# ay-lab/fithic

Measured on AMD Instinct MI355X. Metric: contact-pairs/sec through spline+p-value+BH pass (5 kb cis, whole node), higher is better.
Workload: dtype f64

## Files before the change

### fithic_amd/csrc/fhx_ctx.hpp

```cpp
#pragma once
#include <hip/hip_runtime.h>

#include <atomic>
#include <functional>
#include <chrono>
#include <thread>
#include <memory>
#include <sys/stat.h>
#include <unistd.h>
#include <deque>
#include <mutex>
#include <map>
#include <condition_variable>
#include <algorithm>
#include <climits>
#include <cstddef>
#include <cmath>
#include <cstdio>
#include <cstdlib>
#include <cstring>
#include <string>
#include <vector>

#include "../../include/fithic_mi355x.h"
// ... 42 lines not shown
    const int32_t* loc2;
    const int32_t* count;
    const double* slot_bias;
    bool no_bias;
    const double* prior_lut;
    int lut_len;
    dev::BinomTables intra, inter;
    double inter_chr_prob;
    double outlier_thres;
    int lo_idx, hi_idx;
    int mode;
    int64_t n;
    double* p;
    unsigned long long* top_hist;
    uint8_t* outlier;
    int nonfixed;
    const int32_t* slot_mid;
    const double* table_x;
    const double* table_y;
    int n_table;
    double min_x, max_x;
    long long dist_low, dist_up;
    double total_intra, total_inter;
};

constexpr int K2_THREADS = 256;

constexpr int K2_QUEUES = dev::BC_COUNT - 1;

struct QEntry {
    unsigned int row;
    int count;
    double prior;
};

constexpr int K2_MAX_SHARDS = 2048;

struct QSpan {
    QEntry* base;
    long long cap_s;
    int dir;
    int n_shards;
    const unsigned long long* count;
};
__device__ __forceinline__ QEntry* qentry(const QSpan& q, int shard, long long j) {
    return q.base + (long long)shard * q.cap_s + (long long)q.dir * j;
}

struct K2Queues {
    QSpan q[K2_QUEUES + 1];
    unsigned long long* count;
    unsigned int* heavy_hist;
};

constexpr int K2H_BUCKETS = 2048;
constexpr int K2H_BLOCKS = 1024;
__device__ __forceinline__ int k2h_bucket(int signed_count);

struct CutoffToHost {
    volatile unsigned long long* words = nullptr;
    unsigned long long ticket = 0;
    unsigned int* done = nullptr;
    unsigned long long* zero_me = nullptr;
};

constexpr int K3_DENSE_PERCENT = 35;
constexpr int K2_COUNTER_WORDS = 8;
constexpr int FDR_BUCKETS = 51;

struct DeviceWords {
    unsigned long long bh_kept;
    unsigned long long bh_cutoff;
    unsigned long long bh_below;
    unsigned long long array_kept;
    unsigned long long array_cutoff;
    unsigned long long sort_n;
    unsigned long long run_total;
    unsigned long long nf_keys;
    unsigned long long outliers_added;
    unsigned long long first_dup;
    unsigned long long memo_overflow;
    alignas(128) unsigned long long k2_redo;
    unsigned long long k2_next[K2_COUNTER_WORDS - 1];
    alignas(128) unsigned long long k3_dense;
    alignas(128) unsigned long long fdr_buckets[FDR_BUCKETS];
};
static_assert(offsetof(DeviceWords, k2_next) == offsetof(DeviceWords, k2_redo) + sizeof(unsigned long long) &&
                  sizeof(DeviceWords::k2_next) == (K2_COUNTER_WORDS - 1) * sizeof(unsigned long long),
              "k2_closed zeroes K2_COUNTER_WORDS words starting at k2_redo");
static_assert(K2_COUNTER_WORDS >= 2 + K2_QUEUES, "k2_next holds k2h_heavy's word and one per class queue");
static_assert(sizeof(DeviceWords::fdr_buckets) == FDR_BUCKETS * sizeof(unsigned long long), "one word per FDR bucket");

constexpr int K2_CL_ITEMS = 4;
constexpr int K2_CL_TILE = K2_THREADS * K2_CL_ITEMS;

constexpr int K2_CLOSED = K2_QUEUES + 1;
constexpr int K2_CLOSED_LOCAL = K2_QUEUES + 2;
constexpr int K2_CLASSES = K2_QUEUES + 2;

constexpr int K2H_KCAP = 1023;
constexpr int K2H_GENERIC = 2 * K2H_KCAP;
constexpr int K2H_THREADS = 256;
constexpr int K2H_MAX_ROWS = 4;

constexpr int SORT_THREADS = 256;
constexpr int SORT_WAVES = SORT_THREADS / 64;
constexpr int SORT_ITEMS = 16;
constexpr int SORT_TILE = SORT_THREADS * SORT_ITEMS;
constexpr int CP_THREADS = 1024;
constexpr int CP_WAVES = CP_THREADS / 64;
constexpr int CP_ITEMS = 16;
constexpr int CP_TILE = CP_THREADS * CP_ITEMS;
constexpr int CP_STRIP = 2048;
constexpr int SORT_BLOCKS = 1024;
constexpr int RADIX_BITS = 11;
constexpr int RADIX = 1 << RADIX_BITS;
constexpr int SORT_PASSES = 6;
constexpr int SORT_BITS_LARGE = 8;

constexpr int TOP_SHIFT = 50;
constexpr int TOP_BINS = 8192;

__device__ __forceinline__ unsigned long long pvalue_key(double v) {
    unsigned long long bits = (unsigned long long)__double_as_longlong(v);
    if (bits == 0x8000000000000000ull) bits = 0ull;
    return bits;
}

constexpr unsigned long long KEY_ONE = 0x3FF0000000000000ull;
constexpr unsigned long long KEY_KEEP_ALL = 0x7FF0000000000001ull;

constexpr int SCAT_ITEMS = 8;
constexpr int BH_THREADS = 256;
constexpr int BH_ITEMS = 8;
constexpr int BH_TILE = BH_THREADS * BH_ITEMS;
constexpr int SEG_THREADS = 256;
constexpr int SEG_ITEMS = 16;
constexpr int SEG_TILE = SEG_THREADS * SEG_ITEMS;

}

using namespace fhx;

namespace fhx {
struct DistState;
struct K3Host;
}

struct FhxPinnedPair;
void fhx_pinned_pair_free(FhxPinnedPair* p);

struct SideWorkers {
    std::thread th[2];
    std::mutex mu;
    std::condition_variable cv;
    std::function<void()> job[2];
    bool busy[2] = {false, false}, quit = false, started = false;
    void start() {
        if (started) return;
        started = true;
        for (int k = 0; k < 2; ++k)
            th[k] = std::thread([this, k] {
                std::unique_lock<std::mutex> g(mu);
                for (;;) {
                    cv.wait(g, [&] { return quit || busy[k]; });
                    if (quit) return;
                    std::function<void()> f = std::move(job[k]);
                    g.unlock();
                    f();
                    g.lock();
                    busy[k] = false;
                    cv.notify_all();
                }
// ... 310 lines not shown
```

### fithic_amd/csrc/fhx_k2.hip

```cpp
#include "fhx_ctx.hpp"

namespace fhx {

__device__ __forceinline__ double prior_by_search(const K2Params& P, long long dist) {
    double look = (double)dist;
    if (look < P.min_x) look = P.min_x;
    if (look > P.max_x) look = P.max_x;
    int lo = 0, hi = P.n_table;
    while (lo < hi) {
        const int mid = (lo + hi) >> 1;
        if (P.table_x[mid] < look)
            lo = mid + 1;
        else
            hi = mid;
    }
    return P.table_y[min(lo, P.n_table - 1)];
}

template <int NF = -1>
__device__ __forceinline__ bool row_prior(const K2Params& P, int l1, int l2, double& prior, bool& is_inter) {
    const bool inter = l2 < 0;
    const int s2 = inter ? ~l2 : l2;
    const double b1 = P.no_bias ? 1.0 : P.slot_bias[l1], b2 = P.no_bias ? 1.0 : P.slot_bias[s2];
    if ((b1 < 0 || b2 < 0) && !inter) return false;
// ... 212 lines not shown
            unsigned int mine[2] = {0u, 0u};
            unsigned int shift_of[ITEMS];
#pragma unroll
            for (int r = 0; r < ITEMS; ++r) {
                const int k = cls_of[r] - 1;
                const int f = k >= 3 ? k - 3 : k;
                shift_of[r] = 10u * (unsigned int)(f < 0 ? 0 : f);
                const unsigned int one = k >= 0 ? (1u << shift_of[r]) : 0u;
                mine[0] += k < 3 ? one : 0u;
                mine[1] += k >= 3 ? one : 0u;
            }
            const unsigned int incl0 = wave_incl_sum_u32(mine[0]), incl1 = wave_incl_sum_u32(mine[1]);
            const unsigned int all0 = (unsigned int)__builtin_amdgcn_readlane((int)incl0, 63), all1 = (unsigned int)__builtin_amdgcn_readlane((int)incl1, 63);
            tot[0] = all0 & 1023u; tot[1] = (all0 >> 10) & 1023u; tot[2] = (all0 >> 20) & 1023u;
            tot[3] = all1 & 1023u; tot[4] = (all1 >> 10) & 1023u; tot[5] = (all1 >> 20) & 1023u;
            unsigned int run[2] = {incl0 - mine[0], incl1 - mine[1]};
#pragma unroll
            for (int r = 0; r < ITEMS; ++r) {
                const int k = cls_of[r] - 1;
                const unsigned int word = k >= 3 ? run[1] : run[0];
                before_cls[r] = (word >> shift_of[r]) & 1023u;
                const unsigned int one = k >= 0 ? (1u << shift_of[r]) : 0u;
                run[0] += k < 3 ? one : 0u;
                run[1] += k >= 3 ? one : 0u;
            }
        } else {
#pragma unroll
            for (int r = 0; r < ITEMS; ++r) {
                before_cls[r] = 0;
#pragma unroll
                for (int k = 1; k <= K2_CLASSES; ++k) {
                    const unsigned long long m = __ballot(cls_of[r] == k);
                    if (cls_of[r] == k) before_cls[r] = tot[k - 1] + (unsigned int)__popcll(m & lane_lt);
                    tot[k - 1] += (unsigned int)__popcll(m);
                }
            }
        }
        const unsigned int my_tot = lane == 0 ? tot[0] : (lane == 1 ? tot[1] : (lane == 2 ? tot[2] : (lane == 3 ? tot[3] : tot[4])));
        unsigned int my_base = 0;
        if (lane <= K2_QUEUES && my_tot) my_base = atomicAdd(&cnt[lane], my_tot);
        unsigned int wave_base[K2_QUEUES + 1];
#pragma unroll
        for (int k = 0; k <= K2_QUEUES; ++k) wave_base[k] = __shfl(my_base, k, 64);
#pragma unroll
        for (int r = 0; r < ITEMS; ++r) {
            const int k = cls_of[r] - 1;
            if (k >= 0 && k <= K2_QUEUES) {
                const unsigned int wb = k == 0 ? wave_base[0] : (k == 1 ? wave_base[1] : (k == 2 ? wave_base[2] : (k == 3 ? wave_base[3] : wave_base[4])));
                QEntry e;
                e.row = (unsigned int)(row0 + r);
                e.count = count_of[r];
                e.prior = prior_of[r];
                *qentry(Q.q[k], shard, (long long)(wb + before_cls[r])) = e;
                if (k == dev::BC_CF_SWAPPED - 1 && count_heavy) atomicAdd(&heavy_lds[k2h_bucket(e.count)], 1u);
            } else if (cls_of[r] == K2_CLOSED_LOCAL) {
                cf_prior[wave][before_cls[r]] = prior_of[r];
                cf_idx[wave][before_cls[r]] = (unsigned short)((lane * ITEMS + r) | (count_of[r] < 0 ? 0x8000 : 0));
            }
        }
        __builtin_amdgcn_fence(__ATOMIC_RELEASE, "wavefront");
        __builtin_amdgcn_wave_barrier();
        __builtin_amdgcn_fence(__ATOMIC_ACQUIRE, "wavefront");
        const unsigned int n_local = tot[K2_CLASSES - 1];
        for (unsigned int j = lane; j < n_local; j += 64) {
            const unsigned int ix = cf_idx[wave][j];
            const double n_total = (ix & 0x8000u) ? P.inter.n : P.intra.n;
            const double pr = cf_prior[wave][j];
            const double pv = -dev::cephes_expm1(n_total * dev::cephes_log1p(-pr));
            P.p[wave_row0 + (ix & 0x7FFFu)] = pv;
            H.add(pv);
        }
        __builtin_amdgcn_fence(__ATOMIC_RELEASE, "wavefront");
        __builtin_amdgcn_wave_barrier();
    }
    __syncthreads();
    if (threadIdx.x <= K2_QUEUES) Q.count[(size_t)threadIdx.x * K2_MAX_SHARDS + shard] = cnt[threadIdx.x];
    if (count_heavy)
        for (int d = threadIdx.x; d < K2H_BUCKETS; d += K2_THREADS)
            if (heavy_lds[d]) atomicAdd(&Q.heavy_hist[(size_t)d * K2H_BLOCKS + (shard & (K2H_BLOCKS - 1))], heavy_lds[d]);
    H.flush(P.top_hist);
}

__global__ __launch_bounds__(K2_THREADS) void k2_closed(K2Params P, QSpan q, unsigned long long* __restrict__ zero_words,
                                                        unsigned long long* __restrict__ cutoff_word) {
    __shared__ unsigned int hist_lds[K2_HIST_BINS];
    if (blockIdx.x == 0 && threadIdx.x < K2_COUNTER_WORDS) zero_words[threadIdx.x] = 0ull;
    if (blockIdx.x == 0 && threadIdx.x == K2_COUNTER_WORDS) *cutoff_word = KEY_KEEP_ALL;
    FusedHist H;
    H.init(hist_lds, P.top_hist);
    for (int sh = blockIdx.x; sh < q.n_shards; sh += gridDim.x) {
        const long long n = (long long)q.count[sh];
        for (long long j = threadIdx.x; j < n; j += blockDim.x) {
            const QEntry e = *qentry(q, sh, j);
            const double pv = dev::bdtrc_closed_form(e.count < 0 ? P.inter.n : P.intra.n, e.prior);
            store_p<false>(P.p + e.row, pv);
            H.add(pv);
        }
    }
    H.flush(P.top_hist);
}

struct QDense {
    static constexpr int PAIRS = K2_MAX_SHARDS / 2;
    unsigned int* prefix;
    const unsigned long long* count;
    __device__ __forceinline__ void build(const QSpan& q, unsigned int* prefix_lds, unsigned int* wave_tot) {
        static_assert(PAIRS % K2_THREADS == 0, "whole pairs per thread");
        constexpr int PER = PAIRS / K2_THREADS;
        prefix = prefix_lds;
        count = q.count;
        unsigned int c[PER], s = 0;
#pragma unroll
        for (int k = 0; k < PER; ++k) {
            const int sh = 2 * ((int)threadIdx.x * PER + k);
            c[k] = (sh < q.n_shards ? (unsigned int)q.count[sh] : 0u) + (sh + 1 < q.n_shards ? (unsigned int)q.count[sh + 1] : 0u);
            s += c[k];
        }
        const unsigned int incl = wave_incl_sum_u32(s);
        if ((threadIdx.x & 63) == 63) wave_tot[threadIdx.x >> 6] = incl;
        __syncthreads();
        unsigned int run = incl - s;
        for (int w = 0; w < (int)(threadIdx.x >> 6); ++w) run += wave_tot[w];
#pragma unroll
        for (int k = 0; k < PER; ++k) {
            prefix_lds[threadIdx.x * PER + k] = run;
            run += c[k];
        }
        if (threadIdx.x == K2_THREADS - 1) prefix_lds[PAIRS] = run;
        __syncthreads();
    }
    __device__ __forceinline__ unsigned int total() const { return prefix[PAIRS]; }
    __device__ __forceinline__ int pair_of(unsigned int v) const {
        int lo = 0, hi = PAIRS;
#pragma unroll 1
        while (hi - lo > 1) {
            const int mid = (lo + hi) >> 1;
            if (prefix[mid] <= v)
                lo = mid;
            else
                hi = mid;
        }
        return lo;
    }
    struct Cursor {
        int pr;
        unsigned int base, end, c0;
    };
    __device__ __forceinline__ void load(Cursor& c) const {
        c.base = prefix[c.pr];
        c.end = prefix[c.pr + 1];
        c.c0 = (unsigned int)count[2 * c.pr];
    }
    __device__ __forceinline__ Cursor open(unsigned int v) const {
        Cursor c;
        c.pr = pair_of(v);
        load(c);
        return c;
    }
    __device__ __forceinline__ const QEntry* at(const QSpan& q, Cursor& c, unsigned int v) const {
        if (v >= c.end) {
            do ++c.pr;
            while (v >= prefix[c.pr + 1]);
            load(c);
        }
        const unsigned int u = v - c.base;
        return u < c.c0 ? qentry(q, 2 * c.pr, (long long)u) : qentry(q, 2 * c.pr + 1, (long long)(u - c.c0));
    }
};
constexpr int K2_WAVES = K2_THREADS / 64;

// ... 19 lines not shown
        const bool is_inter = e.count < 0;
        const int c = is_inter ? -e.count : e.count;
        const double pv = dev::bdtrc_count_class<CLS, SMALL_N>(c, is_inter ? P.inter : P.intra, e.prior);
        store_p<false>(P.p + e.row, pv);
        H.add(pv);
    }
    H.flush(P.top_hist);
}

constexpr int K2_SORT_TILE = 1024;
constexpr int K2_SORT_BUCKETS = 32;
template <int CLS, bool SMALL_N, int WPE>
__global__ __launch_bounds__(K2_THREADS) __attribute__((amdgpu_waves_per_eu(WPE))) void k2_queue_by_count(K2Params P, QSpan q,
                                                                                                         unsigned int* next_tile) {
    static_assert(K2_SORT_TILE == 4 * K2_THREADS, "four entries per thread");
    __shared__ QEntry tile[K2_SORT_TILE];
    __shared__ unsigned int bucket_cnt[K2_SORT_BUCKETS], bucket_off[K2_SORT_BUCKETS];
    __shared__ unsigned int hist_lds[K2_HIST_BINS];
    __shared__ unsigned int prefix_lds[QDense::PAIRS + 1], wave_tot[K2_WAVES], tile_lds;
    FusedHist H;
    H.init(hist_lds, P.top_hist);
    QDense D;
    D.build(q, prefix_lds, wave_tot);
    const unsigned int total = D.total();
    const unsigned int share = (total + gridDim.x - 1) / gridDim.x;
    const unsigned int rounds = max(1u, (share + K2_SORT_TILE - 1) / K2_SORT_TILE);
    const unsigned int tile_n = max(min((unsigned int)K2_SORT_TILE, ((share + rounds - 1) / rounds + 63u) & ~63u), 64u);
    const unsigned int tiles = (total + tile_n - 1) / tile_n;
    unsigned int mine = blockIdx.x;
    for (;;) {
        if (threadIdx.x < K2_SORT_BUCKETS) bucket_cnt[threadIdx.x] = 0;
        if (threadIdx.x == 0) tile_lds = mine;
        __syncthreads();
        const unsigned int t = tile_lds;
        if (t >= tiles) break;
        if (threadIdx.x == 0) mine = gridDim.x + atomicAdd(next_tile, 1u);
        const unsigned int v0 = t * tile_n;
        const int m = (int)min(tile_n, total - v0);
        QEntry e[4];
        int bucket[4];
        unsigned int slot[4];
        QDense::Cursor cur{0, 0u, 0u, 0u};
        if ((int)threadIdx.x < m) cur = D.open(v0 + threadIdx.x);
#pragma unroll
        for (int r = 0; r < 4; ++r) {
            const int idx = r * K2_THREADS + (int)threadIdx.x;
            bucket[r] = -1;
            if (idx < m) {
                e[r] = *D.at(q, cur, v0 + idx);
                const int c = e[r].count < 0 ? -e[r].count : e[r].count;
                bucket[r] = c < K2_SORT_BUCKETS - 1 ? c : K2_SORT_BUCKETS - 1;
                slot[r] = atomicAdd(&bucket_cnt[bucket[r]], 1u);
            }
        }
        __syncthreads();
        if (threadIdx.x < K2_SORT_BUCKETS) {
            unsigned int off = 0;
            for (int b = 0; b < (int)threadIdx.x; ++b) off += bucket_cnt[b];
            bucket_off[threadIdx.x] = off;
        }
        __syncthreads();
#pragma unroll
        for (int r = 0; r < 4; ++r)
            if (bucket[r] >= 0) tile[bucket_off[bucket[r]] + slot[r]] = e[r];
        __syncthreads();
#pragma unroll 1
        for (int r = 0; r < 4; ++r) {
            const int idx = r * K2_THREADS + threadIdx.x;
            if (idx < m) {
                const QEntry x = tile[idx];
                const bool is_inter = x.count < 0;
                const int c = is_inter ? -x.count : x.count;
                const double pv = dev::bdtrc_count_class<CLS, SMALL_N>(c, is_inter ? P.inter : P.intra, x.prior);
                store_p<false>(P.p + x.row, pv);
                H.add(pv);
            }
        }
        __syncthreads();
    }
    H.flush(P.top_hist);
}



__device__ __forceinline__ int k2h_bucket(int signed_count) {
    const bool inter = signed_count < 0;
    const int c = inter ? -signed_count : signed_count;
    return c < K2H_KCAP ? (inter ? K2H_KCAP + c : c) : K2H_GENERIC;
}

__global__ __launch_bounds__(K2H_THREADS) void k2h_scatter(QSpan q, const unsigned int* __restrict__ block_hist,
                                                           const unsigned int* __restrict__ off, QEntry* __restrict__ out) {
    __shared__ unsigned int cursor[K2H_BUCKETS];
    for (int d = threadIdx.x; d < K2H_BUCKETS; d += K2H_THREADS) cursor[d] = off[d] + block_hist[(size_t)d * K2H_BLOCKS + blockIdx.x];
    __syncthreads();
    for (int sh = blockIdx.x; sh < q.n_shards; sh += K2H_BLOCKS) {
        const long long n = (long long)q.count[sh];
        for (long long i = threadIdx.x; i < n; i += K2H_THREADS) {
            const QEntry e = *qentry(q, sh, i);
            out[atomicAdd(&cursor[k2h_bucket(e.count)], 1u)] = e;
        }
    }
}

static_assert(dev::kCfIters <= 1024, "one thread per table row");
__device__ __forceinline__ void k2h_table_row(const unsigned int* __restrict__ digit_total, double n_intra, double n_inter,
                                              dev::CfRow* __restrict__ tab) {
    const int b = blockIdx.x;
    if (digit_total[b] == 0 || (int)threadIdx.x >= dev::kCfIters) return;
    const bool inter = b >= K2H_KCAP;
    tab[(size_t)b * dev::kCfIters + threadIdx.x] = dev::cf_swapped_row(inter ? n_inter : n_intra, inter ? b - K2H_KCAP : b, (int)threadIdx.x);
}
__global__ __launch_bounds__(1024) void k2h_offsets_and_tables(const unsigned int* __restrict__ digit_total, unsigned int* __restrict__ off,
                                                               unsigned int granule, double n_intra, double n_inter, dev::CfRow* __restrict__ tab) {
    if (blockIdx.x < K2H_GENERIC) {
        k2h_table_row(digit_total, n_intra, n_inter, tab);
        return;
    }
    __shared__ unsigned int part[1024];
    const unsigned int g1 = granule - 1u;
    const unsigned int a = (digit_total[2 * threadIdx.x] + g1) / granule * granule, b = (digit_total[2 * threadIdx.x + 1] + g1) / granule * granule;
    const int lane = threadIdx.x & 63, wave = threadIdx.x >> 6;
    const unsigned int incl = wave_incl_sum_u32(a + b);
    if (lane == 63) part[wave] = incl;
    __syncthreads();
    unsigned int excl = incl - (a + b);
    for (int w = 0; w < wave; ++w) excl += part[w];
    if (threadIdx.x == 1023) off[K2H_BUCKETS] = excl + a + b;
    off[2 * threadIdx.x] = excl;
    off[2 * threadIdx.x + 1] = excl + a;
}


struct K2HeavyParams {
    dev::BinomTables intra, inter;
    double* p;
    unsigned long long* top_hist;
};
__device__ unsigned long long g_k2h_clk[4];

template <int R, int WPE, bool SMALL_N>
__global__ __launch_bounds__(K2H_THREADS) __attribute__((amdgpu_waves_per_eu(WPE, WPE))) void k2h_heavy(
    K2HeavyParams P, const QEntry* __restrict__ sorted, const unsigned int* __restrict__ off,
    const unsigned int* __restrict__ digit_total, const dev::CfRow* __restrict__ tab, QEntry* __restrict__ redo,
    unsigned long long* __restrict__ n_redo, unsigned int* __restrict__ next_task) {
    static_assert(R >= 1 && R <= K2H_MAX_ROWS, "the sorted queue is padded for at most K2H_MAX_ROWS rows per lane");
    __shared__ unsigned int hist_lds[K2_HIST_BINS];
    FusedHist H;
    H.init(hist_lds, P.top_hist);
    const int wave = __builtin_amdgcn_readfirstlane((int)(threadIdx.x >> 6));
    const int lane = threadIdx.x & 63;
    constexpr unsigned int TASK = 64u * R;
    const unsigned int n_tasks = off[K2H_GENERIC] / TASK;
    const unsigned int n_waves = gridDim.x * (K2H_THREADS / 64);
    if (blockIdx.x == 0 && threadIdx.x == 0) {
        g_k2h_clk[0] = __builtin_amdgcn_s_memtime();
        g_k2h_clk[1] = __builtin_amdgcn_s_memrealtime();
    }
    for (unsigned int task = blockIdx.x * (K2H_THREADS / 64) + wave; task < n_tasks;) {
        const unsigned int first = task * TASK;
        int lo = 0, hi = K2H_GENERIC;
        while (hi - lo > 1) {
            const int mid = (lo + hi) >> 1;
            if (off[mid] <= first)
                lo = mid;
            else
                hi = mid;
        }
        const int b = __builtin_amdgcn_readfirstlane(lo);
        const unsigned int live = off[b] + digit_total[b];
        const bool is_inter = b >= K2H_KCAP;
        const int c = is_inter ? b - K2H_KCAP : b;
        const dev::BinomTables& T = is_inter ? P.inter : P.intra;
        const double fk = (double)c - 1.0;
        const double aa = fk + 1.0, bb = T.n - fk;
        QEntry e[R];
        bool have[R], irregular[R];
        double w1[R], cf[R];
#pragma unroll
        for (int r = 0; r < R; ++r) {
            const unsigned int j = first + (unsigned int)r * 64u + (unsigned int)lane;
            have[r] = j < live;
            e[r].row = 0u;
            e[r].count = is_inter ? -c : c;
            e[r].prior = 0.5;
            if (have[r]) e[r] = sorted[j];
            w1[r] = 1.0 - e[r].prior;
            irregular[r] = !have[r] || !dev::cf_swapped_regular(bb, aa, w1[r]);
        }
        const dev::CfRowConstPtr rows = (dev::CfRowConstPtr)(uintptr_t)(tab + (size_t)b * dev::kCfIters);
        dev::cf_swapped_uniform<R>(rows, w1, irregular, cf);
#pragma unroll
        for (int r = 0; r < R; ++r) {
            double pv = 0.0;
            const bool mine = have[r] && !irregular[r];
            if (have[r]) {
                if (__builtin_expect(irregular[r], 0))
                    redo[atomicAdd(n_redo, 1ull)] = e[r];
                else {
                    pv = dev::incbet_finish<SMALL_N>(bb, aa, w1[r], e[r].prior, cf[r], 1, T.lbeta[c], (SMALL_N && T.small_n) ? T.inv_beta[c] : 0.0);
                    store_p<true>(P.p + e[r].row, pv);
                }
            }
            H.add_wave_min(pv, mine);
        }
        unsigned int next = 0;
        if (lane == 0) next = atomicAdd(next_task, 1u);
        task = n_waves + (unsigned int)__builtin_amdgcn_readfirstlane((int)next);
    }
    if (blockIdx.x == 0 && threadIdx.x == 0) {
        g_k2h_clk[2] = __builtin_amdgcn_s_memtime();
        g_k2h_clk[3] = __builtin_amdgcn_s_memrealtime();
    }
    H.flush(P.top_hist);
}

__global__ __launch_bounds__(K2_THREADS) void k2h_generic(K2Params P, const QEntry* __restrict__ sorted,
                                                          const unsigned int* __restrict__ off,
                                                          const unsigned int* __restrict__ digit_total,
                                                          const QEntry* __restrict__ redo,
                                                          const unsigned long long* __restrict__ n_redo) {
    const QEntry* base = sorted + off[K2H_GENERIC];
    const int64_t n_generic = (int64_t)digit_total[K2H_GENERIC];
    const int64_t n = n_generic + (int64_t)*n_redo;
    __shared__ unsigned int hist_lds[K2_HIST_BINS];
    FusedHist H;
    H.init(hist_lds, P.top_hist);
    const int64_t stride = (int64_t)gridDim.x * blockDim.x;
    for (int64_t j = (int64_t)blockIdx.x * blockDim.x + threadIdx.x; j < n; j += stride) {
        const QEntry e = j < n_generic ? base[j] : redo[j - n_generic];
        const bool is_inter = e.count < 0;
        const int c = is_inter ? -e.count : e.count;
        const double pv = dev::bdtrc_count_class<dev::BC_CF_SWAPPED>(c, is_inter ? P.inter : P.intra, e.prior);
        store_p<true>(P.p + e.row, pv);
        H.add(pv);
    }
    H.flush(P.top_hist);
}


__global__ void k_debug_classify(double n_total, const int32_t* __restrict__ count, const double* __restrict__ prior, int64_t n,
                                 int32_t* __restrict__ by_table, int32_t* __restrict__ by_arith, double* __restrict__ thr5) {
    const int64_t i = (int64_t)blockIdx.x * blockDim.x + threadIdx.x;
    if (i >= n) return;
    const dev::ClsRow r = dev::cls_row(n_total, count[i]);
    by_table[i] = dev::cls_is_trivial(count[i], n_total, prior[i]) ? (int)dev::BC_TRIVIAL : dev::cls_lookup(r, prior[i]);
    by_arith[i] = dev::bdtrc_class(count[i], n_total, prior[i]);
    if (thr5) {
        thr5[5 * i] = r.tA;
        thr5[5 * i + 1] = r.tB;
        thr5[5 * i + 2] = r.tC;
        thr5[5 * i + 3] = r.tD;
        thr5[5 * i + 4] = r.tE;
    }
}

__global__ void k_outlier_flags(const double* __restrict__ p, double thres, int64_t n, uint8_t* __restrict__ flags) {
    const int64_t stride = (int64_t)gridDim.x * blockDim.x;
    for (int64_t i = (int64_t)blockIdx.x * blockDim.x + threadIdx.x; i < n; i += stride) flags[i] = (p[i] < thres) ? 1 : 0;
}

__global__ __launch_bounds__(fhxscan::THREADS) void k_flag_count(const unsigned char* __restrict__ flag, int64_t n, unsigned int* __restrict__ tile_counts) {
    const int64_t base = (int64_t)blockIdx.x * fhxscan::TILE + (int64_t)threadIdx.x * fhxscan::SCAN_ITEMS;
    unsigned int c = 0;
    for (int k = 0; k < fhxscan::SCAN_ITEMS; ++k)
        if (base + k < n && flag[base + k]) ++c;
    unsigned int total;
    fhxscan::block_exclusive_scan(c, &total);
    if (threadIdx.x == 0) tile_counts[blockIdx.x] = total;
}
__global__ __launch_bounds__(fhxscan::THREADS) void k_flag_rows(const unsigned char* __restrict__ flag, int64_t n,
                                                                 const unsigned long long* __restrict__ tile_offsets, int64_t* __restrict__ rows) {
    const int64_t base = (int64_t)blockIdx.x * fhxscan::TILE + (int64_t)threadIdx.x * fhxscan::SCAN_ITEMS;
    unsigned int c = 0;
    for (int k = 0; k < fhxscan::SCAN_ITEMS; ++k)
        if (base + k < n && flag[base + k]) ++c;
    unsigned int total;
    unsigned long long at = tile_offsets[blockIdx.x] + fhxscan::block_exclusive_scan(c, &total);
    for (int k = 0; k < fhxscan::SCAN_ITEMS; ++k)
        if (base + k < n && flag[base + k]) rows[at++] = base + k;
}

__global__ void k_bdtrc_array(dev::BinomTables T, const int32_t* __restrict__ count, const double* __restrict__ prior,
                              int64_t n, double* __restrict__ out) {
    const int64_t stride = (int64_t)gridDim.x * blockDim.x;
    for (int64_t i = (int64_t)blockIdx.x * blockDim.x + threadIdx.x; i < n; i += stride)
        out[i] = dev::bdtrc_count(count[i], T, prior[i]);
}

template <int KIND, int LAZY>
__global__ void k_debug_contfrac(const double* __restrict__ a, const double* __restrict__ b, const double* __restrict__ x,
                                 int64_t n, double* __restrict__ out) {
    const int64_t stride = (int64_t)gridDim.x * blockDim.x;
    for (int64_t i = (int64_t)blockIdx.x * blockDim.x + threadIdx.x; i < n; i += stride)
        out[i] = LAZY ? dev::contfrac_lazy<KIND>(a[i], b[i], x[i]) : dev::contfrac<KIND>(a[i], b[i], x[i]);
}
// ... 204 lines not shown
    if (allow_memo && !ctx->have_bias && !ctx->nonfixed && !getenv("FHX_NO_MEMO")) {
        plan.memo_nd = plan.memo_intra ? (int)(P.hi_idx - P.lo_idx + 1) : 0;
        const int64_t budget = std::min<int64_t>(1ll << 24, ctx->n_rows / 4);
        const int64_t per_count = (int64_t)plan.memo_nd + (plan.memo_inter ? 1 : 0);
        if (per_count > 0 && plan.memo_nd >= 0) {
            const int64_t cap = std::min<int64_t>(ctx->stats.max_count, budget / per_count - 1);
            if (cap >= 8) plan.memo_cap = (int)cap;
        }
    }
    plan.k2_n = plan.memo_cap < 0 ? ctx->n_rows : (int64_t)plan.memo_nd * (plan.memo_cap + 1) + (plan.memo_inter ? (plan.memo_cap + 1) : 0);
    plan.small_n = (P.intra.small_n && P.intra.n >= 1.0) || (P.inter.small_n && P.inter.n >= 1.0);
    plan.legacy_heavy = getenv("FHX_K2_LEGACY") != nullptr;
    const char* heavy_rows_env = plan.legacy_heavy ? nullptr : std::getenv("FHX_K2H_ROWS");
    const int heavy_rows = heavy_rows_env ? std::atoi(heavy_rows_env) : 0;
    plan.heavy_rows = (heavy_rows == 2 || heavy_rows == 4) ? heavy_rows
                      : plan.k2_n < 32000000 ? 2 : 4;
    plan.cap_s = k2_shard_capacity(plan.k2_n);
    plan.n_shards = k2_classify_grid(plan.k2_n);
    return plan;
}

struct K2Memo {
    int32_t *loc1 = nullptr, *loc2 = nullptr, *count = nullptr;
    double* table = nullptr;
    unsigned int* over_rows = nullptr;
    unsigned long long over_cap = 0;
};
static int k2_table_rows(fhx_ctx* ctx, const K2Plan& plan, K2Memo* M, K2Params* P) {
    M->over_cap = (unsigned long long)std::max<int64_t>(ctx->n_rows / 16, 1024);
    const size_t col = ((size_t)plan.k2_n + 3) / 4 * 4;
    const size_t need = col * (4 + 4 + 4 + 8) + (size_t)M->over_cap * 4 + 64;
    if (need > ctx->memo_bytes) {
        dev_free(ctx->d_memo);
        ctx->memo_bytes = 0;
        FHX_HIP(hipMalloc(&ctx->d_memo, need));
        ctx->memo_bytes = need;
    }
    M->loc1 = reinterpret_cast<int32_t*>(ctx->d_memo);
    M->loc2 = M->loc1 + col;
    M->count = M->loc2 + col;
    M->table = reinterpret_cast<double*>(M->count + col);
    M->over_rows = reinterpret_cast<unsigned int*>(M->table + col);
    hipLaunchKernelGGL(k2_memo_rows, dim3(grid_for(plan.k2_n, 256)), dim3(256), 0, ctx->stream, plan.memo_nd, P->lo_idx, plan.memo_cap,
                       (int)plan.memo_inter, M->loc1, M->loc2, M->count, plan.k2_n);
    P->loc1 = M->loc1;
    P->loc2 = M->loc2;
    P->count = M->count;
    P->p = M->table;
    P->n = plan.k2_n;
    return FHX_OK;
}

static int k2_queue_layout(fhx_ctx* ctx, const K2Plan& plan, bool prezeroed, K2Queues* Q) {
    if ((int64_t)plan.n_shards * plan.cap_s > ctx->queue_cap) return fail(ctx, FHX_ERR_HIP, "internal: queue workspace smaller than the shard layout");
    if (!ctx->d_k2_counts) FHX_HIP(hipMalloc(&ctx->d_k2_counts, (size_t)(K2_QUEUES + 1) * K2_MAX_SHARDS * sizeof(unsigned long long)));
    Q->count = ctx->d_k2_counts;
    static_assert((K2H_BLOCKS & (K2H_BLOCKS - 1)) == 0, "shard -> column by masking");
    Q->heavy_hist = plan.legacy_heavy ? nullptr : ctx->d_block_hist;
    if (Q->heavy_hist && !prezeroed)
        FHX_HIP(hipMemsetAsync(ctx->d_block_hist, 0, (size_t)K2H_BUCKETS * K2H_BLOCKS * sizeof(unsigned int), ctx->stream));
    ctx->k2_shards = plan.n_shards;
    auto span = [&](int cls, QEntry* buf, int dir) {
        Q->q[cls - 1] = QSpan{dir > 0 ? buf : buf + plan.cap_s - 1, plan.cap_s, dir, plan.n_shards, Q->count + (size_t)(cls - 1) * K2_MAX_SHARDS};
    };
    span(dev::BC_CF_SWAPPED, ctx->d_queue[0], 1);
    span(dev::BC_PSERIES, ctx->d_queue[0], -1);
    span(dev::BC_CF_BCF, ctx->d_queue[1], 1);
    span(dev::BC_CF_BD, ctx->d_queue[1], -1);
    span(K2_CLOSED, ctx->d_queue_sorted, 1);
    return FHX_OK;
}

template <int CLS, bool SMALL_N>
static void launch_k2_queue(fhx_ctx* ctx, const K2Params& P, const K2Queues& Q) {
    hipLaunchKernelGGL(HIP_KERNEL_NAME(k2_queue<CLS, SMALL_N>), dim3(2 * resident_grid(ctx, k2_queue<CLS, SMALL_N>)), dim3(K2_THREADS), 0,
                       ctx->stream, P, Q.q[CLS - 1]);
}
template <int CLS, bool SMALL_N>
static void launch_k2_queue_by_count(fhx_ctx* ctx, const K2Params& P, const K2Queues& Q) {
    constexpr int PIECE = SMALL_N ? 4 : 5;
    hipLaunchKernelGGL(HIP_KERNEL_NAME(k2_queue_by_count<CLS, SMALL_N, PIECE>), dim3(resident_grid(ctx, k2_queue_by_count<CLS, SMALL_N, PIECE>)),
                       dim3(K2_THREADS), 0, ctx->stream, P, Q.q[CLS - 1], (unsigned int*)(ctx->d_words->k2_next + CLS));
}
template <int ROWS, int WAVES, bool SMALL_N>
static void launch_k2h_heavy(fhx_ctx* ctx, const K2Params& P, QEntry* redo) {
    hipLaunchKernelGGL(HIP_KERNEL_NAME(k2h_heavy<ROWS, WAVES, SMALL_N>), dim3(256 * WAVES), dim3(K2H_THREADS), 0, ctx->stream,
                       K2HeavyParams{P.intra, P.inter, P.p, P.top_hist}, (const QEntry*)ctx->d_queue_sorted, (const unsigned int*)ctx->d_k2h_off,
                       (const unsigned int*)ctx->d_digit_total, (const dev::CfRow*)ctx->d_cf_tab, redo, &ctx->d_words->k2_redo,
                       (unsigned int*)ctx->d_words->k2_next);
}

template <bool SMALL_N>
static int launch_k2(fhx_ctx* ctx, const K2Plan& plan, const K2Params& P, const K2Queues& Q) {
    const dim3 cgrid(plan.n_shards), block(K2_THREADS);
    if (P.nonfixed)
        hipLaunchKernelGGL(HIP_KERNEL_NAME(k2_classify<1, 4, 0>), cgrid, block, 0, ctx->stream, P, Q);
    else
        hipLaunchKernelGGL(HIP_KERNEL_NAME(k2_classify<0, 4, 3, true, true>), cgrid, block, 0, ctx->stream, P, Q);
    hipLaunchKernelGGL(k2_closed, dim3(256 * 8), block, 0, ctx->stream, P, Q.q[K2_CLOSED - 1], &ctx->d_words->k2_redo, &ctx->d_words->bh_cutoff);
    if (plan.legacy_heavy) {
        FHX_HIP(hipEventRecord(ctx->ev[6], ctx->stream));
        launch_k2_queue<dev::BC_CF_SWAPPED, SMALL_N>(ctx, P, Q);
        FHX_HIP(hipEventRecord(ctx->ev[7], ctx->stream));
        ctx->ev_folded[3] = false;
        launch_k2_queue_by_count<dev::BC_CF_BD, SMALL_N>(ctx, P, Q);
        launch_k2_queue_by_count<dev::BC_CF_BCF, SMALL_N>(ctx, P, Q);
        launch_k2_queue<dev::BC_PSERIES, SMALL_N>(ctx, P, Q);
        return FHX_OK;
    }
    static_assert(K2H_BUCKETS == RADIX && K2H_BLOCKS == SORT_BLOCKS, "the radix sort's count matrix and scan are reused");
    QEntry* hq = ctx->d_queue[0];
    launch_rs_scan(ctx, (int)SORT_BLOCKS);
    hipLaunchKernelGGL(k2h_offsets_and_tables, dim3(K2H_GENERIC + 1), dim3(1024), 0, ctx->stream, (const unsigned int*)ctx->d_digit_total,
                       ctx->d_k2h_off, 64u * (unsigned int)plan.heavy_rows, P.intra.n, P.inter.n, ctx->d_cf_tab);
    hipLaunchKernelGGL(k2h_scatter, dim3(K2H_BLOCKS), dim3(K2H_THREADS), 0, ctx->stream, Q.q[dev::BC_CF_SWAPPED - 1],
                       (const unsigned int*)ctx->d_block_hist, (const unsigned int*)ctx->d_k2h_off, ctx->d_queue_sorted);
    launch_k2_queue<dev::BC_PSERIES, SMALL_N>(ctx, P, Q);
    FHX_HIP(hipEventRecord(ctx->ev[6], ctx->stream));
    if (plan.heavy_rows == 2) launch_k2h_heavy<2, 8, SMALL_N>(ctx, P, hq);
    else launch_k2h_heavy<4, 4, SMALL_N>(ctx, P, hq);
    FHX_HIP(hipEventRecord(ctx->ev[7], ctx->stream));
    ctx->ev_folded[3] = false;
    hipLaunchKernelGGL(k2h_generic, dim3(256 * 4), dim3(K2_THREADS), 0, ctx->stream, P, (const QEntry*)ctx->d_queue_sorted,
                       (const unsigned int*)ctx->d_k2h_off, (const unsigned int*)ctx->d_digit_total, (const QEntry*)hq,
                       (const unsigned long long*)&ctx->d_words->k2_redo);
    launch_k2_queue_by_count<dev::BC_CF_BD, SMALL_N>(ctx, P, Q);
    launch_k2_queue_by_count<dev::BC_CF_BCF, SMALL_N>(ctx, P, Q);
    return FHX_OK;
}

static int k2_fused_hist(fhx_ctx* ctx, bool prezeroed, K2Params* P) {
    if (!ctx->d_k2_hist) FHX_HIP(hipMalloc(&ctx->d_k2_hist, TOP_BINS * sizeof(unsigned long long)));
    if (!prezeroed) FHX_HIP(hipMemsetAsync(ctx->d_k2_hist, 0, TOP_BINS * sizeof(unsigned long long), ctx->stream));
    P->top_hist = ctx->d_k2_hist;
    return FHX_OK;
}

static int run_k2(fhx_ctx* ctx, const K2Plan& plan, const K2Params& P, bool prezeroed) {
    K2Queues Q;
    const int rc = k2_queue_layout(ctx, plan, prezeroed, &Q);
    if (rc != FHX_OK) return rc;
    return plan.small_n ? launch_k2<true>(ctx, plan, P, Q) : launch_k2<false>(ctx, plan, P, Q);
}

static int finish_k2(fhx_ctx* ctx, const K2Plan& plan, const K2Params& P_rows, const K2Memo& M) {
    if (plan.memo_cap >= 0) {
        unsigned long long* n_over = &ctx->d_words->memo_overflow;
        FHX_HIP(hipMemsetAsync(n_over, 0, sizeof(unsigned long long), ctx->stream));
        hipLaunchKernelGGL(k2_memo_gather, dim3(grid_for(ctx->n_rows, 256, 256 * 16)), dim3(256), 0, ctx->stream, P_rows, (const double*)M.table,
                           plan.memo_nd, plan.memo_cap, (int)plan.memo_intra, (int)plan.memo_inter, M.over_rows, n_over, M.over_cap);
        FHX_HIP(hipGetLastError());
        unsigned long long h_over = 0;
        FHX_HIP(hipMemcpyAsync(&h_over, n_over, sizeof(h_over), hipMemcpyDeviceToHost, ctx->stream));
        FHX_HIP(hipStreamSynchronize(ctx->stream));
        if (h_over > 0) {
            const bool listed = h_over <= M.over_cap;
            const int64_t work = listed ? (int64_t)h_over : ctx->n_rows;
            hipLaunchKernelGGL(k2_memo_overflow, dim3(grid_for(work, 256, 256 * 16)), dim3(256), 0, ctx->stream, P_rows,
                               (const unsigned int*)M.over_rows, (int64_t)h_over, listed ? 1 : 0);
            FHX_HIP(hipGetLastError());
            FHX_HIP(hipStreamSynchronize(ctx->stream));
        }
    }
    FHX_HIP(hipGetLastError());
    FHX_HIP(hipEventRecord(ctx->ev[3], ctx->stream));
    ctx->ev_valid[1] = true;
    ctx->ev_folded[1] = false;
    ctx->have_p = true;
    ctx->have_q = false;
    ctx->n_sorted = -1;
    return FHX_OK;
}

int fhx_pvalues(fhx_ctx* ctx) {
    if (!ctx) return FHX_ERR_ARG;
    if (ctx->device < 0) return fail(ctx, FHX_ERR_NO_DEVICE, "host-only context");
    if (!ctx->have_fit) return fail(ctx, FHX_ERR_ARG, "fhx_fit must run first");
    FHX_HIP(hipSetDevice(ctx->device));
    if (ctx->tables_dirty) {
        const int r2 = build_slot_tables(ctx);
        if (r2 != FHX_OK) return r2;
    }
    K2Params P = make_k2_params(ctx);
    before_rerecord(ctx, 1);
    FHX_HIP(hipEventRecord(ctx->ev[2], ctx->stream));
    const K2Plan plan = plan_k2(ctx, P);
    const bool prezeroed = ctx->k2_prezeroed;
    ctx->k2_prezeroed = false;
    ctx->k2_hist_valid = false;
    if (plan.memo_cap < 0) {
        const int rh = k2_fused_hist(ctx, prezeroed, &P);
        if (rh != FHX_OK) return rh;
        ctx->k2_hist_valid = true;
    }
    const K2Params P_rows = P;
    K2Memo M;
    int rc = plan.memo_cap >= 0 ? k2_table_rows(ctx, plan, &M, &P) : FHX_OK;
    if (rc == FHX_OK) rc = run_k2(ctx, plan, P, prezeroed);
    return rc == FHX_OK ? finish_k2(ctx, plan, P_rows, M) : rc;
}

int fhx_bdtrc_array(fhx_ctx* ctx, double n_total, const int32_t* count, const double* prior, int64_t n, double* out) {
    if (!ctx || !count || !prior || !out || n < 0) return FHX_ERR_ARG;
    if (ctx->device < 0) return fail(ctx, FHX_ERR_NO_DEVICE, "host-only context");
    if (n == 0) return FHX_OK;
    FHX_HIP(hipSetDevice(ctx->device));
    if (std::fabs(n_total) < 9.2e18 && n_total == std::floor(n_total)) n_total = bdtrc_total(ctx->prm, (long long)n_total);
    int64_t mc = 1;
    for (int64_t i = 0; i < n; ++i) mc = std::max<int64_t>(mc, count[i]);
    std::vector<double> lb, ib;
// ... 398 lines not shown
```

Baseline: 13.84 billion.

## Fold BD/BCF count-class tiles into the persistent k2h_heavy kernel tail

The separate per-class launches for the BC_CF_BD and BC_CF_BCF queues are replaced by a shared tile loop. In the 4-row path it runs at the end of a persistent, resident-grid k2h_heavy kernel; in the 2-row path it runs in a new standalone k2_converging kernel. k2_closed now publishes the two queue spans into device words so the fused code can find them. Work is handed out through one ticket counter that carries over from the first class into the second. The aim is to cut launches and idle tail time between the heavy and count-class phases. In exchange, the heavy kernel uses more LDS, which can lower its occupancy, and its grid size and task-counter wiring change. A profiling timeline script is also added.

After: 13.96 billion, median of 6. About the same (+0.9%).

```diff
diff --git a/fithic_amd/csrc/fhx_ctx.hpp b/fithic_amd/csrc/fhx_ctx.hpp
--- a/fithic_amd/csrc/fhx_ctx.hpp
+++ b/fithic_amd/csrc/fhx_ctx.hpp
@@ -148,6 +148,7 @@
     unsigned long long memo_overflow;
     alignas(128) unsigned long long k2_redo;
     unsigned long long k2_next[K2_COUNTER_WORDS - 1];
+    alignas(128) QSpan k2_conv[2];
     alignas(128) unsigned long long k3_dense;
     alignas(128) unsigned long long fdr_buckets[FDR_BUCKETS];
 };
@@ -155,6 +156,9 @@
                   sizeof(DeviceWords::k2_next) == (K2_COUNTER_WORDS - 1) * sizeof(unsigned long long),
               "k2_closed zeroes K2_COUNTER_WORDS words starting at k2_redo");
 static_assert(K2_COUNTER_WORDS >= 2 + K2_QUEUES, "k2_next holds k2h_heavy's word and one per class queue");
+constexpr int K2_CONV_WORD = 16;
+static_assert(offsetof(DeviceWords, k2_conv) == offsetof(DeviceWords, k2_redo) + K2_CONV_WORD * sizeof(unsigned long long),
+              "k2_conv sits K2_CONV_WORD words behind k2_redo");
 static_assert(sizeof(DeviceWords::fdr_buckets) == FDR_BUCKETS * sizeof(unsigned long long), "one word per FDR bucket");
 
 constexpr int K2_CL_ITEMS = 4;
diff --git a/fithic_amd/csrc/fhx_k2.hip b/fithic_amd/csrc/fhx_k2.hip
--- a/fithic_amd/csrc/fhx_k2.hip
+++ b/fithic_amd/csrc/fhx_k2.hip
@@ -318,10 +318,15 @@
 }
 
 __global__ __launch_bounds__(K2_THREADS) void k2_closed(K2Params P, QSpan q, unsigned long long* __restrict__ zero_words,
-                                                        unsigned long long* __restrict__ cutoff_word) {
+                                                        unsigned long long* __restrict__ cutoff_word, QSpan conv_bd, QSpan conv_bcf) {
     __shared__ unsigned int hist_lds[K2_HIST_BINS];
     if (blockIdx.x == 0 && threadIdx.x < K2_COUNTER_WORDS) zero_words[threadIdx.x] = 0ull;
     if (blockIdx.x == 0 && threadIdx.x == K2_COUNTER_WORDS) *cutoff_word = KEY_KEEP_ALL;
+    if (blockIdx.x == 0 && threadIdx.x == K2_COUNTER_WORDS + 1) {
+        QSpan* conv = reinterpret_cast<QSpan*>(zero_words + K2_CONV_WORD);
+        conv[0] = conv_bd;
+        conv[1] = conv_bcf;
+    }
     FusedHist H;
     H.init(hist_lds, P.top_hist);
     for (int sh = blockIdx.x; sh < q.n_shards; sh += gridDim.x) {
@@ -507,6 +512,94 @@
 }
 
 
+struct K2TileLds {
+    QEntry tile[K2_SORT_TILE];
+    unsigned int bucket_cnt[K2_SORT_BUCKETS], bucket_off[K2_SORT_BUCKETS];
+    unsigned int prefix[QDense::PAIRS + 1], wave_tot[K2_WAVES], ticket;
+};
+template <int CLS, bool SMALL_N>
+__device__ __forceinline__ unsigned int k2_class_tiles(const dev::BinomTables& intra, const dev::BinomTables& inter, double* __restrict__ p,
+                                                       FusedHist& H, const QSpan& q, unsigned int* next_tile, K2TileLds& S,
+                                                       unsigned int mine, unsigned int& base) {
+    static_assert(K2_SORT_TILE == 4 * K2_THREADS, "four entries per thread");
+    QDense D;
+    D.build(q, S.prefix, S.wave_tot);
+    const unsigned int total = D.total();
+    const unsigned int share = (total + gridDim.x - 1) / gridDim.x;
+    const unsigned int rounds = max(1u, (share + K2_SORT_TILE - 1) / K2_SORT_TILE);
+    const unsigned int tile_n = max(min((unsigned int)K2_SORT_TILE, ((share + rounds - 1) / rounds + 63u) & ~63u), 64u);
+    const unsigned int tiles = (total + tile_n - 1) / tile_n;
+    unsigned int t;
+    for (;;) {
+        if (threadIdx.x < K2_SORT_BUCKETS) S.bucket_cnt[threadIdx.x] = 0;
+        if (threadIdx.x == 0) S.ticket = mine;
+        __syncthreads();
+        t = S.ticket;
+        if (t - base >= tiles) break;
+        if (threadIdx.x == 0) mine = gridDim.x + atomicAdd(next_tile, 1u);
+        const unsigned int v0 = (t - base) * tile_n;
+        const int m = (int)min(tile_n, total - v0);
+        QEntry e[4];
+        int bucket[4];
+        unsigned int slot[4];
+        QDense::Cursor cur{0, 0u, 0u, 0u};
+        if ((int)threadIdx.x < m) cur = D.open(v0 + threadIdx.x);
+#pragma unroll
+        for (int r = 0; r < 4; ++r) {
+            const int idx = r * K2_THREADS + (int)threadIdx.x;
+            bucket[r] = -1;
+            if (idx < m) {
+                e[r] = *D.at(q, cur, v0 + idx);
+                const int c = e[r].count < 0 ? -e[r].count : e[r].count;
+                bucket[r] = c < K2_SORT_BUCKETS - 1 ? c : K2_SORT_BUCKETS - 1;
+                slot[r] = atomicAdd(&S.bucket_cnt[bucket[r]], 1u);
+            }
+        }
+        __syncthreads();
+        if (threadIdx.x < K2_SORT_BUCKETS) {
+            unsigned int off = 0;
+            for (int b = 0; b < (int)threadIdx.x; ++b) off += S.bucket_cnt[b];
+            S.bucket_off[threadIdx.x] = off;
+        }
+        __syncthreads();
+#pragma unroll
+        for (int r = 0; r < 4; ++r)
+            if (bucket[r] >= 0) S.tile[S.bucket_off[bucket[r]] + slot[r]] = e[r];
+        __syncthreads();
+#pragma unroll 1
+        for (int r = 0; r < 4; ++r) {
+            const int idx = r * K2_THREADS + threadIdx.x;
+            if (idx < m) {
+                const QEntry x = S.tile[idx];
+                const bool is_inter = x.count < 0;
+                const int c = is_inter ? -x.count : x.count;
+                const double pv = dev::bdtrc_count_class<CLS, SMALL_N>(c, is_inter ? inter : intra, x.prior);
+                store_p<false>(p + x.row, pv);
+                H.add(pv);
+            }
+        }
+        __syncthreads();
+    }
+    base += tiles;
+    return t;
+}
+template <bool SMALL_N>
+__device__ __forceinline__ void k2_converging_tiles(const dev::BinomTables& intra, const dev::BinomTables& inter, double* __restrict__ p,
+                                                    FusedHist& H, unsigned long long* k2_words, K2TileLds& S) {
+    const QSpan* conv = reinterpret_cast<const QSpan*>(k2_words + K2_CONV_WORD);
+    unsigned int* next_tile = reinterpret_cast<unsigned int*>(k2_words + 1 + dev::BC_CF_BD);
+    unsigned int base = 0;
+    unsigned int t = blockIdx.x;
+    {
+        const QSpan q = conv[0];
+        t = k2_class_tiles<dev::BC_CF_BD, SMALL_N>(intra, inter, p, H, q, next_tile, S, t, base);
+    }
+    {
+        const QSpan q = conv[1];
+        k2_class_tiles<dev::BC_CF_BCF, SMALL_N>(intra, inter, p, H, q, next_tile, S, t, base);
+    }
+}
+
 
 __device__ __forceinline__ int k2h_bucket(int signed_count) {
     const bool inter = signed_count < 0;
@@ -564,13 +657,15 @@
 };
 __device__ unsigned long long g_k2h_clk[4];
 
-template <int R, int WPE, bool SMALL_N>
+template <int R, int WPE, bool SMALL_N, bool MERGED = false>
 __global__ __launch_bounds__(K2H_THREADS) __attribute__((amdgpu_waves_per_eu(WPE, WPE))) void k2h_heavy(
     K2HeavyParams P, const QEntry* __restrict__ sorted, const unsigned int* __restrict__ off,
     const unsigned int* __restrict__ digit_total, const dev::CfRow* __restrict__ tab, QEntry* __restrict__ redo,
     unsigned long long* __restrict__ n_redo, unsigned int* __restrict__ next_task) {
     static_assert(R >= 1 && R <= K2H_MAX_ROWS, "the sorted queue is padded for at most K2H_MAX_ROWS rows per lane");
+    static_assert(!MERGED || K2H_THREADS == K2_THREADS, "phase B is written for K2_THREADS threads");
     __shared__ unsigned int hist_lds[K2_HIST_BINS];
+    if (MERGED) next_task = reinterpret_cast<unsigned int*>(n_redo + 1);
     FusedHist H;
     H.init(hist_lds, P.top_hist);
     const int wave = __builtin_amdgcn_readfirstlane((int)(threadIdx.x >> 6));
@@ -637,6 +732,21 @@
         g_k2h_clk[2] = __builtin_amdgcn_s_memtime();
         g_k2h_clk[3] = __builtin_amdgcn_s_memrealtime();
     }
+    if constexpr (MERGED) {
+        __shared__ K2TileLds tile_lds;
+        __syncthreads();
+        k2_converging_tiles<SMALL_N>(P.intra, P.inter, P.p, H, n_redo, tile_lds);
+    }
+    H.flush(P.top_hist);
+}
+template <bool SMALL_N>
+__global__ __launch_bounds__(K2_THREADS) __attribute__((amdgpu_waves_per_eu(4, 4))) void k2_converging(K2HeavyParams P,
+                                                                                                      unsigned long long* k2_words) {
+    __shared__ unsigned int hist_lds[K2_HIST_BINS];
+    __shared__ K2TileLds tile_lds;
+    FusedHist H;
+    H.init(hist_lds, P.top_hist);
+    k2_converging_tiles<SMALL_N>(P.intra, P.inter, P.p, H, k2_words, tile_lds);
     H.flush(P.top_hist);
 }
 
@@ -1007,6 +1117,24 @@
     hipLaunchKernelGGL(HIP_KERNEL_NAME(k2_queue_by_count<CLS, SMALL_N, PIECE>), dim3(resident_grid(ctx, k2_queue_by_count<CLS, SMALL_N, PIECE>)),
                        dim3(K2_THREADS), 0, ctx->stream, P, Q.q[CLS - 1], (unsigned int*)(ctx->d_words->k2_next + CLS));
 }
+static int k2_conv_grid(int resident) {
+    const char* env = std::getenv("FHX_K2_GRID");
+    const int want = env ? std::atoi(env) : 0;
+    return want >= 1 && want < resident ? want : resident;
+}
+template <int ROWS, int WAVES, bool SMALL_N>
+static void launch_k2_merged(fhx_ctx* ctx, const K2Params& P, QEntry* redo) {
+    auto kernel = k2h_heavy<ROWS, WAVES, SMALL_N, true>;
+    hipLaunchKernelGGL(kernel, dim3(k2_conv_grid(resident_grid(ctx, kernel))), dim3(K2H_THREADS), 0, ctx->stream,
+                       K2HeavyParams{P.intra, P.inter, P.p, P.top_hist}, (const QEntry*)ctx->d_queue_sorted, (const unsigned int*)ctx->d_k2h_off,
+                       (const unsigned int*)ctx->d_digit_total, (const dev::CfRow*)ctx->d_cf_tab, redo, &ctx->d_words->k2_redo,
+                       (unsigned int*)nullptr);
+}
+template <bool SMALL_N>
+static void launch_k2_converging(fhx_ctx* ctx, const K2Params& P) {
+    hipLaunchKernelGGL(HIP_KERNEL_NAME(k2_converging<SMALL_N>), dim3(k2_conv_grid(resident_grid(ctx, k2_converging<SMALL_N>))),
+                       dim3(K2_THREADS), 0, ctx->stream, K2HeavyParams{P.intra, P.inter, P.p, P.top_hist}, &ctx->d_words->k2_redo);
+}
 template <int ROWS, int WAVES, bool SMALL_N>
 static void launch_k2h_heavy(fhx_ctx* ctx, const K2Params& P, QEntry* redo) {
     hipLaunchKernelGGL(HIP_KERNEL_NAME(k2h_heavy<ROWS, WAVES, SMALL_N>), dim3(256 * WAVES), dim3(K2H_THREADS), 0, ctx->stream,
@@ -1022,7 +1150,8 @@
         hipLaunchKernelGGL(HIP_KERNEL_NAME(k2_classify<1, 4, 0>), cgrid, block, 0, ctx->stream, P, Q);
     else
         hipLaunchKernelGGL(HIP_KERNEL_NAME(k2_classify<0, 4, 3, true, true>), cgrid, block, 0, ctx->stream, P, Q);
-    hipLaunchKernelGGL(k2_closed, dim3(256 * 8), block, 0, ctx->stream, P, Q.q[K2_CLOSED - 1], &ctx->d_words->k2_redo, &ctx->d_words->bh_cutoff);
+    hipLaunchKernelGGL(k2_closed, dim3(256 * 8), block, 0, ctx->stream, P, Q.q[K2_CLOSED - 1], &ctx->d_words->k2_redo, &ctx->d_words->bh_cutoff,
+                       Q.q[dev::BC_CF_BD - 1], Q.q[dev::BC_CF_BCF - 1]);
     if (plan.legacy_heavy) {
         FHX_HIP(hipEventRecord(ctx->ev[6], ctx->stream));
         launch_k2_queue<dev::BC_CF_SWAPPED, SMALL_N>(ctx, P, Q);
@@ -1043,14 +1172,13 @@
     launch_k2_queue<dev::BC_PSERIES, SMALL_N>(ctx, P, Q);
     FHX_HIP(hipEventRecord(ctx->ev[6], ctx->stream));
     if (plan.heavy_rows == 2) launch_k2h_heavy<2, 8, SMALL_N>(ctx, P, hq);
-    else launch_k2h_heavy<4, 4, SMALL_N>(ctx, P, hq);
+    else launch_k2_merged<4, 4, SMALL_N>(ctx, P, hq);
     FHX_HIP(hipEventRecord(ctx->ev[7], ctx->stream));
     ctx->ev_folded[3] = false;
     hipLaunchKernelGGL(k2h_generic, dim3(256 * 4), dim3(K2_THREADS), 0, ctx->stream, P, (const QEntry*)ctx->d_queue_sorted,
                        (const unsigned int*)ctx->d_k2h_off, (const unsigned int*)ctx->d_digit_total, (const QEntry*)hq,
                        (const unsigned long long*)&ctx->d_words->k2_redo);
-    launch_k2_queue_by_count<dev::BC_CF_BD, SMALL_N>(ctx, P, Q);
-    launch_k2_queue_by_count<dev::BC_CF_BCF, SMALL_N>(ctx, P, Q);
+    if (plan.heavy_rows == 2) launch_k2_converging<SMALL_N>(ctx, P);
     return FHX_OK;
 }
 
diff --git a/profiles/k2_timeline.py b/profiles/k2_timeline.py
--- /dev/null
+++ b/profiles/k2_timeline.py
@@ -0,0 +1,44 @@
+#!/usr/bin/env python3
+import sqlite3
+import sys
+
+db = sqlite3.connect(sys.argv[1])
+n_pass = int(sys.argv[2]) if len(sys.argv) > 2 else 5
+cur = db.cursor()
+tabs = [r[0] for r in cur.execute("select name from sqlite_master where type='table'")]
+ks = [t for t in tabs if t.startswith("rocpd_info_kernel_symbol")][0]
+kd = [t for t in tabs if t.startswith("rocpd_kernel_dispatch")][0]
+rows = list(cur.execute("select s.kernel_name, d.start, d.end from %s d join %s s on d.kernel_id=s.id order by d.start" % (kd, ks)))
+
+
+def short(name):
+    return name.split("(")[0].replace("void ", "").replace("fhx::", "")[:44]
+
+
+def is_k2(name):
+    return any(k in name for k in ("k2_", "k2h_", "rs_scan"))
+
+
+starts = [i for i, r in enumerate(rows) if "k2_classify" in r[0]][-n_pass:]
+if not starts:
+    sys.exit("no k2_classify dispatch among %d dispatches; first names: %s" % (len(rows), [r[0][:60] for r in rows[:5]]))
+acc = {}
+spans = []
+for p, i0 in enumerate(starts):
+    j = i0
+    while j + 1 < len(rows) and is_k2(rows[j + 1][0]) and "k2_classify" not in rows[j + 1][0]:
+        j += 1
+    seg = rows[i0:j + 1]
+    t0, prev_end = seg[0][1], None
+    print("pass -%d" % (len(starts) - p))
+    for k, (name, a, b) in enumerate(seg):
+        gap = (a - prev_end) / 1e3 if prev_end is not None else 0.0
+        print("  %9.1f us  gap %+7.1f us  %8.1f us  %s" % ((a - t0) / 1e3, gap, (b - a) / 1e3, short(name)))
+        acc.setdefault((k, short(name)), []).append((gap, (b - a) / 1e3))
+        prev_end = max(prev_end or b, b)
+    spans.append((prev_end - t0) / 1e3)
+    print("  K2 span %.1f us" % spans[-1])
+print("mean over %d passes" % len(starts))
+for (k, name), v in sorted(acc.items()):
+    print("  gap %+7.1f us  %8.1f us  %s" % (sum(g for g, _ in v) / len(v), sum(d for _, d in v) / len(v), name))
+print("  K2 span %.1f us (min %.1f, max %.1f)" % (sum(spans) / len(spans), min(spans), max(spans)))
```
